# chhylp123/BitMapperBS

Hardware: AMD Instinct MI355X
Metric: M 150bp PE reads aligned/s (higher is better)
Workload: dtype u64

## Files before the change

### bitmapperbs_amd/csrc/bmbs_api.hip

```cpp
#include "bmbs_host.h"
#include "bmbs_kernels.hip"



int ensure(Lane* c, DevBuf& b, size_t bytes, bool zero)
{
    if (bytes == 0) bytes = 16;
    if (b.cap >= bytes) return BMBS_OK;
    size_t want = bytes + bytes / 8 + 256;
    if (c->kn.arena && want <= ((size_t)256 << 20)) {
        if (b.cap) want = std::min<size_t>(std::max(want, b.cap + b.cap / 2), (size_t)256 << 20);
        void* p = c->arena.alloc(want);
        if (!p) { c->err = "out of device memory (lane arena)"; return BMBS_ENOMEM; }
        if (b.p && !b.arena) (void)hipFree(b.p);
        b.p = p; b.cap = want; b.arena = true;
    } else {
        if (b.p && !b.arena) (void)hipFree(b.p);
        b.p = nullptr; b.cap = 0; b.arena = false;
        hipError_t e = hipMalloc(&b.p, want);
        if (e != hipSuccess) { c->err = std::string("hipMalloc: ") + hipGetErrorString(e); b.p = nullptr; return BMBS_ENOMEM; }
        b.cap = want;
    }
    if (zero && hipMemsetAsync(b.p, 0, want, c->stream) != hipSuccess) { c->err = "hipMemsetAsync failed"; return BMBS_ESTATE; }
    return BMBS_OK;
// ... 916 lines not shown
    prof_begin(c, "k_reduce");
    HIPCHK(c, hipMemsetAsync(st.job_flag, 0, n * 4, c->stream));
    HIPCHK(c, hipMemsetAsync(st.red_status, 0, n, c->stream));
    hipLaunchKernelGGL(k_reduce, dim3(nblk(n, 256)), dim3(256), 0, c->stream, (long)n, c->prm.ambiguous_out, st, c->vote_off.as<u64>(),
                       c->votes_dense.as<bmbs_vote>(), c->ferr.as<u32>(), c->fend.as<int>(), tot_at(c, TOT_VOTE_READS), c->vote_list.as<u32>());
    prof_end(c);
    return BMBS_OK;
}

int map_se_dev(Lane* c, const Pending& P)
{
    ReadGeom gm = {};
    int max_ops = 0;
    int rc = call_open(c, P, (u64)P.n, &gm, &max_ops);
    if (rc || P.n == 0) return rc;
    const u64 n = (u64)P.n;
    const char* d_seq = reinterpret_cast<const char*>(P.a[0]);
    const char* d_qual = reinterpret_cast<const char*>(P.a[1]);
    if (P.packed_hw) {
        ENS(c, c->pk_ascii, n * (u64)P.stride + 64);
        { int rz_ = ensure(c, c->prow, n * (u64)pack_words(gm.L) * 8 + 64, true); if (rz_) return rz_; } ENS(c, c->prow_dirty, n + 64);
        HIPCHK(c, hipMemsetAsync(c->prow_dirty.p, 0, n + 64, c->stream));
        prof_begin(c, "k_rows_from_packed");
        rows_from_packed(c, reinterpret_cast<const u64*>(P.a[0]), P.packed_hw, gm, 0, n, false, c->pk_ascii.as<char>(), P.stride);
        prof_end(c);
        d_seq = c->pk_ascii.as<char>();
    }
    const ReadState st = read_state(c);
    u64 tot = 0;
    rc = run_seed_stages(c, d_seq, gm, P.stride, n, &tot, 0, P.exact, P.packed_hw > 0);
    if (rc) return rc;
    c->last_total_cand = tot;
    rc = se_filter_reduce(c, gm, st, d_seq, P.stride, n, tot, P.exact);
    if (rc) return rc;
    rc = align_jobs(c, P, gm, st, d_seq, d_qual, nullptr, n, 0xffffffffu, max_ops);
    if (rc) return rc;
    prof_begin(c, "k_finalize");
    hipLaunchKernelGGL(k_finalize, dim3(nblk(n, 256)), dim3(256), 0, c->stream, c->ix, c->sp, c->pen_lut.as<int>(),
                       c->mapq_lut.as<u8>(), c->mapq_off.as<u32>(), c->mapq_unit, d_seq, d_qual, gm, P.stride, (long)n, st, c->a_start.as<int>(),
                       c->a_end.as<int>(), c->a_nm.as<u32>(), c->a_score.as<int>(), c->a_nops.as<int>(), max_ops, P.cigar_base,
                       c->prm.ambiguous_out, c->sd_sp0.as<u64>(), c->sd_hits0.as<u32>(),
                       reinterpret_cast<bmbs_result_dev*>(P.d_results), c->call_stats.as<unsigned long long>());
    prof_end(c);
    return call_end(c, P.slot);
}

struct PeCall {
    Lane* c; ReadGeom gm; PeIns pi; ReadState st; PeState ps; PeCand *A, *B; char* seq_all; u64 n, n2; int stride; bool exact; u64 tot;
    bool prepacked;
    int rows(const Pending& P);
    int seed();
    int votes();
    int verify_round(int round, u64 cap, const char* name_f, const char* name_c);
    int verify_fast();
    int verify_sensitive();
};

int PeCall::rows(const Pending& P)
{
    prepacked = false;
    if (P.packed_hw) {
        { int rz_ = ensure(c, c->prow, n2 * (u64)pack_words(gm.L) * 8 + 64, true); if (rz_) return rz_; } ENS(c, c->prow_dirty, n2 + 64);
        HIPCHK(c, hipMemsetAsync(c->prow_dirty.p, 0, n2 + 64, c->stream));
        prof_begin(c, "k_rows_from_packed");
        rows_from_packed(c, reinterpret_cast<const u64*>(P.a[0]), P.packed_hw, gm, 0, n, false, seq_all, stride);
        rows_from_packed(c, reinterpret_cast<const u64*>(P.a[2]), P.packed_hw, gm, n, n, true, seq_all, stride);
        prof_end(c);
        prepacked = true;
    } else if (!P.prepared) {
        u64* prow = nullptr; u32* pdirty = nullptr;
        const int pwords = pack_words(gm.L), W = pack_base_words(gm.L);
        if (use_packed_rows(c)) {
            { int rz_ = ensure(c, c->prow, n2 * (u64)pwords * 8 + 64, true); if (rz_) return rz_; } ENS(c, c->prow_dirty, n2 + 64);
            HIPCHK(c, hipMemsetAsync(c->prow_dirty.p, 0, n2 + 64, c->stream));
            prow = c->prow.as<u64>(); pdirty = c->prow_dirty.as<u32>(); prepacked = true;
        }
        const int sparse = prow != nullptr;
        const char* seq1 = reinterpret_cast<const char*>(P.a[0]);
        const char* seq2 = reinterpret_cast<const char*>(P.a[2]);
        prof_begin(c, "k_pe_prepare");
        const int ppr = stride / 16;
        if (sparse && ppr <= 256) {
            const int rpb = 256 / ppr;
            hipLaunchKernelGGL(k_pe_prepare_p, dim3(std::min<u64>(nblk(n, rpb), 2048)), dim3(256), (size_t)rpb * (ppr + 1) * 16, c->stream,
                               seq1, seq2, gm, stride, (long)n, seq_all, prow, pwords, W, pdirty);
        } else
        hipLaunchKernelGGL(k_pe_prepare, dim3(nblk(n * (stride / 16), 256)), dim3(256), 0, c->stream, seq1, seq2, gm, stride, (long)n, seq_all,
                           prow, pwords, W, pdirty, sparse);
        prof_end(c);
    }
    return BMBS_OK;
}

int PeCall::seed()
{
    ps.occ = c->pe_occ.as<int>(); ps.len = c->pe_len.as<u32>(); ps.cur = c->pe_cur.as<u8>(); ps.vround = c->pe_vround.as<u8>();
    ps.dead = c->pe_dead.as<u8>(); ps.both = c->pe_both.as<u8>(); ps.npair = c->pe_npair.as<int>(); ps.sbd = c->pe_sbd.as<u32>();
    if (c->prm.sensitive) {
        ENS(c, c->pe_first, n); ENS(c, c->pe_full, n2); ENS(c, c->pe_roff, n2 * 8); ENS(c, c->pe_rflag, n * 4); ENS(c, c->pe_rscan, (n + 1) * 8);
        ENS(c, c->pe_rlist, n * 4); ENS(c, c->pe_rcnt, n * 4); ENS(c, c->pe_ritem_off, (n + 1) * 8);
    }
    ps.first = c->pe_first.as<u8>(); ps.full = c->pe_full.as<u8>(); ps.R = c->pe_R.as<PeCand>(); ps.roff = c->pe_roff.as<u64>();
    c->last_reseeded = 0; c->last_reseed_cand = 0;
    int rc = launch_seeding(c, seq_all, gm, stride, n2, 1, prepacked);
    if (rc) return rc;
    prof_begin(c, "scan_cand");
// ... 24 lines not shown
        hipLaunchKernelGGL(k_vote_pe_dense, dim3(nblk(n2, VOTE_DENSE_BLOCK)), dim3(VOTE_DENSE_BLOCK), 0, c->stream, c->ix, (long)n2, gm, st, ps, A, c->long_flag.as<u32>(), mid_flag);
    else
        hipLaunchKernelGGL(k_vote_pe_fused, dim3(nblk(n2, 64)), dim3(64), 0, c->stream, c->ix, (long)n2, gm, st, ps, A, c->long_flag.as<u32>(), mid_flag);
    prof_end(c);
    if (use_mid) {
        prof_begin(c, "k_vote_pe_mid");
        int rc = scan_u32(c, mid_flag, n2, c->long_off.as<u64>(), TOT_MID, c->pe_mid_list.as<u32>());
        if (rc) return rc;
        hipLaunchKernelGGL(k_vote_pe_mid, dim3(nblk(n2, 64)), dim3(64), 0, c->stream, c->ix, gm, st, ps, tot_at(c, TOT_MID), c->pe_mid_list.as<u32>(), A, cnt);
        prof_end(c);
    }
    prof_begin(c, "k_vote_pe_long");
    const int prefilter = (!c->prm.sensitive && c->kn.prefilter) ? 1 : 0;
    int rc = scan_u32(c, c->long_flag.as<u32>(), n2, c->long_off.as<u64>(), TOT_LONG, c->long_list.as<u32>());
    if (rc) return rc;
    ENS(c, c->big_list, n2 * 4 + 64);
    unsigned long long* big_count = c->totals.as<unsigned long long>() + TOT_BIG;
    HIPCHK(c, hipMemsetAsync(big_count, 0, 8, c->stream));
    hipLaunchKernelGGL((k_vote_pe_long<VM_CAP, VM_BLOCK, VOTE_REG>), dim3(32768), dim3(VM_BLOCK), 0, c->stream, c->ix, gm, st, ps,
                       tot_at(c, TOT_LONG), c->long_list.as<u32>(), A, c->big_list.as<u32>(), big_count, c->cand.as<u64>(), cnt, (long)n, pi, prefilter, c->long_flag.as<u32>());
    prof_end(c);
    prof_begin(c, "k_vote_pe_big");
    hipLaunchKernelGGL((k_vote_pe_long<1024, 128, VM_CAP>), dim3(8192), dim3(128), 0, c->stream, c->ix, gm, st, ps,
                       tot_at(c, TOT_BIG), c->big_list.as<u32>(), A, (u32*)nullptr, (unsigned long long*)nullptr, c->cand.as<u64>(), cnt, (long)n, pi, prefilter, c->long_flag.as<u32>());
    hipLaunchKernelGGL((k_vote_pe_long<2048, 256, 1024>), dim3(4096), dim3(256), 0, c->stream, c->ix, gm, st, ps,
                       tot_at(c, TOT_BIG), c->big_list.as<u32>(), A, (u32*)nullptr, (unsigned long long*)nullptr, c->cand.as<u64>(), cnt, (long)n, pi, prefilter, c->long_flag.as<u32>());
    hipLaunchKernelGGL((k_vote_pe_long<VL_CAP, VL_BLOCK, 2048>), dim3(2048), dim3(VL_BLOCK), 0, c->stream, c->ix, gm, st, ps,
                       tot_at(c, TOT_BIG), c->big_list.as<u32>(), A, (u32*)nullptr, (unsigned long long*)nullptr, c->cand.as<u64>(), cnt, (long)n, pi, prefilter, c->long_flag.as<u32>());
    prof_end(c);
    return BMBS_OK;
}

int PeCall::verify_round(int round, u64 cap, const char* name_f, const char* name_c)
{
    if (cap) {
        prof_begin(c, name_f);
        u32* wcnt = c->sd_flag_c.as<u32>();
        u64* woff = c->sd_off_c.as<u64>();
        hipLaunchKernelGGL(k_pe_count, dim3(nblk(n2, 256)), dim3(256), 0, c->stream, (long)n, (long)n2, round, ps, wcnt);
        int rc = scan_u32(c, wcnt, n2, woff, TOT_PE_WORK);
        if (rc) return rc;
        hipLaunchKernelGGL(k_pe_worklist, dim3(nblk(n2, 256)), dim3(256), 0, c->stream, (long)n2, wcnt, woff, c->dense_read.as<u32>(),
                           c->ferr.as<u32>());
        hipLaunchKernelGGL(k_filter_pe, dim3(nblk(cap, 256)), dim3(256), 0, c->stream, c->ix, seq_all, packed_rows(c, gm), gm, stride, st, ps, A, B,
                           tot_at(c, TOT_PE_WORK), c->dense_read.as<u32>(), c->ferr.as<u32>(), c->counters.as<unsigned long long>());
        prof_end(c);
    }
    prof_begin(c, name_c);
    hipLaunchKernelGGL(k_pe_compact, dim3(nblk(n2, 64)), dim3(64), 0, c->stream, (long)n, (long)n2, gm, round, st, ps, A, B);
    prof_end(c);
    return BMBS_OK;
}

int PeCall::verify_fast()
{
    prof_begin(c, "k_pe_filter_pairs");
    u32* pef_flag = (c->kn.pef_long == 2 || (c->kn.pef_long == 1 && c->lr_long > 0.005)) ? c->long_flag.as<u32>() : nullptr;
    if (pef_flag) HIPCHK(c, hipMemsetAsync(pef_flag, 0, n * 4, c->stream));
    hipLaunchKernelGGL(k_pe_filter_pairs, dim3(nblk(n, 64)), dim3(64), 0, c->stream, (long)n, gm, pi, st, ps, A, B, pef_flag,
                       c->counters.as<unsigned long long>());
    if (pef_flag) {
        int rc = scan_u32(c, pef_flag, n, c->long_off.as<u64>(), TOT_PEF_LONG, c->long_list.as<u32>());
        if (rc) return rc;
        hipLaunchKernelGGL(k_pe_filter_pairs_long, dim3((unsigned)std::min<u64>(n, 65536)), dim3(64), 0, c->stream, (long)n, gm, pi, st, ps, tot_at(c, TOT_PEF_LONG),
                           c->long_list.as<u32>(), A, B);
    }
    prof_end(c);
    int rc = verify_round(1, tot, "k_filter_pe_r1", "k_pe_compact_r1");
    if (rc) return rc;
    prof_begin(c, "k_pe_prune");
    hipLaunchKernelGGL(k_pe_prune, dim3(nblk(n, 64)), dim3(64), 0, c->stream, (long)n, gm, pi, st, ps, A, B);
    prof_end(c);
    return verify_round(2, tot, "k_filter_pe_r2", "k_pe_compact_r2");
}

int PeCall::verify_sensitive()
{
    unsigned long long* cnt = c->counters.as<unsigned long long>();
    prof_begin(c, "k_pes_order");
    hipLaunchKernelGGL(k_pes_order, dim3(nblk(n, 256)), dim3(256), 0, c->stream, (long)n, st, seed_carry(c), ps);
    prof_end(c);
    int rc = verify_round(1, tot, "k_filter_pe_r1", "k_pe_compact_r1");
    if (rc) return rc;
    prof_begin(c, "k_pes_second");
    hipLaunchKernelGGL(k_pes_second, dim3(nblk(n, 64)), dim3(64), 0, c->stream, (long)n, gm, pi, st, ps, A, B);
    prof_end(c);
    rc = verify_round(2, tot, "k_filter_pe_r2", "k_pe_compact_r2");
    if (rc) return rc;
    prof_begin(c, "k_pes_reseed");
    u32* rflag = c->pe_rflag.as<u32>();
    u32* rlist = c->pe_rlist.as<u32>();
    u32* rcnt = c->pe_rcnt.as<u32>();
    u64* n_reseed = tot_at(c, TOT_RESEED);
    hipLaunchKernelGGL(k_pes_reseed_flag, dim3(nblk(n, 256)), dim3(256), 0, c->stream, (long)n, ps, rflag);
    rc = scan_u32(c, rflag, n, c->pe_rscan.as<u64>(), TOT_RESEED, rlist);
    if (rc) return rc;
    HIPCHK(c, hipMemsetAsync(rcnt, 0, n * 4, c->stream));
    {
        const PackedRows prs = packed_rows(c, gm);
        const bool kg = c->ix.occ3 && prs.base && (c->kn.kgram >= 2 || (c->kn.kgram == 1 && c->lr_chain >= 3.0));
        hipLaunchKernelGGL((kg ? k_pes_reseed<true, true> : prs.base ? k_pes_reseed<true> : k_pes_reseed<false>), dim3(nblk(n, 64)), dim3(64), 0, c->stream, c->ix, seq_all, prs, gm, stride,
                           (long)n, n_reseed, rlist, st, ps, rcnt, cnt);
    }
    rc = scan_u32(c, rcnt, n, c->pe_ritem_off.as<u64>(), TOT_RCAND);
    if (rc) return rc;
    prof_end(c);
    u64 rt[2] = {0, 0};
    if (exact) {
        HIPCHK(c, hipMemcpyAsync(rt, tot_at(c, TOT_RESEED), sizeof rt, hipMemcpyDeviceToHost, c->stream));
        HIPCHK(c, hipStreamSynchronize(c->stream));
    } else {
        rt[0] = n; rt[1] = cap_from(c->lr_rcand, n2, c->kn.cap_scale < 1.0 ? 64 : 65536, c->kn.cap_scale);
        hipLaunchKernelGGL(k_guard_rcand, dim3(nblk(n, 256)), dim3(256), 0, c->stream, tot_at(c, TOT_RCAND), rt[1], c->flags.as<u32>(), (long)n, rcnt,
                           c->pe_ritem_off.as<u64>());
        hipLaunchKernelGGL(k_guard_done, dim3(1), dim3(1), 0, c->stream, tot_at(c, TOT_RCAND), c->flags.as<u32>(), BMBS_FLAG_RCAND);
    }
    c->last_reseeded = rt[0]; c->last_reseed_cand = rt[1];
    if (!rt[0]) return BMBS_OK;
    const u64 rtot = exact ? std::max<u64>(rt[1], cap_from((double)rt[1] / (double)n2, n2, 65536)) : (rt[1] ? rt[1] : 1);
    ENS(c, c->pe_R, rtot * sizeof(PeCand)); ENS(c, c->pe_rcand, rtot * 8);
    ENS(c, c->dense_read, rtot * 4); ENS(c, c->ferr, rtot * 4);
    ps.R = c->pe_R.as<PeCand>();
    prof_begin(c, "k_pes_vote");
    u32* pv_flag = c->long_flag.as<u32>();
    hipLaunchKernelGGL(k_pes_vote, dim3(nblk(rt[0], 64)), dim3(64), 0, c->stream, c->ix, (long)n, gm, pi, n_reseed, rlist,
                       c->pe_ritem_off.as<u64>(), st, ps, c->pe_rcand.as<u64>(), A, B, pv_flag, cnt);
// ... 901 lines not shown
```

### bitmapperbs_amd/csrc/bmbs_host.h

```cpp
#ifndef BMBS_HOST_H
#define BMBS_HOST_H
#include "../../include/bmbs.h"
#include "bmbs_dev.h"
#include <algorithm>
#include <atomic>
#include <cmath>
#include <cstdio>
#include <cstring>
#include <ctime>
#include <sys/syscall.h>
#include <unistd.h>
#include <deque>
#include <memory>
#include <mutex>
#include <string>
#include <thread>
#include <vector>


struct DevBuf {
    void* p = nullptr; size_t cap = 0;
    bool arena = false;
    template <class T> T* as() const { return reinterpret_cast<T*>(p); }
};

struct Arena {
    struct Slab { char* p; size_t cap, used; };
    std::vector<Slab> slabs;
    size_t total = 0;
    void* alloc(size_t bytes)
    {
        bytes = (bytes + 255) & ~(size_t)255;
        for (size_t i = slabs.size(); i-- > 0;)
            if (slabs[i].used + bytes <= slabs[i].cap) { void* r = slabs[i].p + slabs[i].used; slabs[i].used += bytes; return r; }
        size_t cap = std::max<size_t>(bytes, std::min<size_t>((size_t)2 << 30, std::max<size_t>((size_t)512 << 20, total / 2)));
        void* p = nullptr;
        if (hipMalloc(&p, cap) != hipSuccess) {
            cap = bytes;
            if (hipMalloc(&p, cap) != hipSuccess) return nullptr;
        }
        slabs.push_back({(char*)p, cap, bytes});
        total += cap;
        return p;
    }
    void free_all() { for (auto& s : slabs) (void)hipFree(s.p); slabs.clear(); total = 0; }
};

struct Prof { const char* name; hipEvent_t a, b; bool used; };

struct Knobs {
    int sw_form = 0;
    bool rows_ascii = false;
    int seed_waves = 65536;
    bool exact = false;
    int lanes = 3;
    int host_lanes = 4;
    long chunk = 0;
    long split_min = 250000;
    int up_turns = 1;
    int scan_chain = 0;
    int prefilter = 1;
    int pef_long = 1;
    int vote_dense = 1;
    int kgram = 1;
    int seed_stage = 1;
    double cap_scale = 1.0;
    static const bool copy_streams = true, copy_lock = true, arena = true;
    void read()
    {
        auto is = [](const char* e, const char* v) { return e && !strcmp(e, v); };
        const char* e = getenv("BMBS_SW");
        sw_form = is(e, "reg") ? 1 : is(e, "reg2") ? 2 : is(e, "wave") ? 3 : 0;
        rows_ascii = is(getenv("BMBS_LEGACY"), "1");
        if ((e = getenv("BMBS_SEED_WAVES"))) seed_waves = atoi(e);
        exact = is(getenv("BMBS_EXACT"), "1");
        if ((e = getenv("BMBS_LANES"))) lanes = atoi(e);
        if (lanes < 1) lanes = 1;
        if (lanes > 8) lanes = 8;
        if ((e = getenv("BMBS_HOST_LANES"))) host_lanes = atoi(e);
        if (host_lanes < lanes) host_lanes = lanes;
        if (host_lanes > 8) host_lanes = 8;
        if ((e = getenv("BMBS_KGRAM"))) kgram = atoi(e);
        if ((e = getenv("BMBS_CHUNK"))) chunk = atol(e);
        if ((e = getenv("BMBS_SPLIT_MIN"))) split_min = atol(e);
        if (split_min < 1) split_min = 1;
        if ((e = getenv("BMBS_CAP_SCALE"))) cap_scale = atof(e);
        if ((e = getenv("BMBS_PEF_LONG"))) pef_long = atoi(e);
        if ((e = getenv("BMBS_PREFILTER"))) prefilter = atoi(e);
        if ((e = getenv("BMBS_VOTE_DENSE"))) vote_dense = atoi(e);
        if ((e = getenv("BMBS_UP_TURNS"))) up_turns = atoi(e);
        if ((e = getenv("BMBS_SCAN_CHAIN"))) scan_chain = atoi(e);
        if ((e = getenv("BMBS_SEED_STAGE"))) seed_stage = atoi(e) == 0 ? 0 : 1;
    }
};

struct Pending {
    bool pe = false, exact = false;
    int slot = 0;
    uint64_t a[4] = {0, 0, 0, 0};
    const u16* d_len = nullptr;
    int32_t L = 0, stride = 0;
    int64_t n = 0;
    uint64_t d_results = 0, d_cigar_pool = 0;
    int64_t cigar_cap = 0;
    u32 cigar_base = 0;
    bool prepared = false;
    int packed_hw = 0;
    bool staged = false;
};

struct Occ3Shared {
    std::mutex mu;
    bool tried = false;
    int skipped = 0;
    int dev = 0;
    DevIndex base;
    u64 rows = 0;
    void* occ3 = nullptr; void* c3 = nullptr; u64 nb3 = 0;
    ~Occ3Shared() { if (occ3 || c3) { (void)hipSetDevice(dev); if (occ3) (void)hipFree(occ3); if (c3) (void)hipFree(c3); } }
};

struct RecIn { DevBuf in, len, off; };

struct Lane {
    int dev = 0;
    hipStream_t stream = nullptr;
    hipStream_t up_stream = nullptr, down_stream = nullptr;
    hipEvent_t ev_up = nullptr, ev_k = nullptr;
    bmbs_params prm;
    ScoreParams sp;
    Knobs kn;
    Arena arena;
    std::string err;
    bool attached = false;
    DevIndex ix;
    u64 rows = 0;
    DevBuf occ, hash, sa, gen2, gen2p, chrom_start, t20;
    std::shared_ptr<Occ3Shared> o3;
    DevBuf pen_lut, mapq_lut;
    bool luts_ready = false;
    int mapq_unit = 0;
    DevBuf mapq_off, klut;
// ... 143 lines not shown
```

### bitmapperbs_amd/csrc/k_pe_fast.hip

```cpp
struct PeCand { u64 site; u32 err; int32_t end; };

struct PeIns { int min_ins, max_ins; };
DEVI void pe_bounds(const ReadGeom& gm, const PeIns& pi, long p, long n, long long& maxd, long long& mind, int& large_k)
{
    const int L1 = gm.rl(p), L2 = gm.rl(p + n);
    const int k1 = gm.rk(L1), k2 = gm.rk(L2);
    large_k = k1 > k2 ? k1 : k2;
    maxd = (long long)pi.max_ins + 2LL * large_k;
    mind = (long long)pi.min_ins - 2LL * large_k - (L1 > L2 ? L1 : L2);
}

struct PeState {
    int*  occ;
    u32*  len;
    u8*   cur;
    u8*   vround;
    u8*   dead;
    u8*   both;
    int*  npair;
    u32*  sbd;
    u8*   first;
    u8*   full;
    PeCand* R;
    u64*  roff;
// ... 416 lines not shown
                if (mate_here && turn == 0) __threadfence();
                __syncthreads();
                continue;
            }
            vl_locate_range(ix, st.seeds + (size_t)r * BMBS_MAX_SEEDS, st.n_seeds[r], 0, (int)nc, keys, sh_pref, true);
            int cnt = (int)nc;
            if (prefilter && v == 3) {
                const bool earlier = !listed(m) || (long)st.n_cand[m] <= LO;
                const bool mate_final = (turn == 1 || earlier) && ps.len[m] <= PREF_STAGE;
                long long maxd, mind; int large_k;
                pe_bounds(gm, pi, r < n_pairs ? r : r - n_pairs, n_pairs, maxd, mind, large_k);
                if (mate_final && mind <= 0 && maxd >= 0) {
                    const int occm = ps.occ[m];
                    const long nm = occm == 0 ? 0 : (long)ps.len[m];
                    const PeCand* ml = A + st.cand_off[m];
                    if (nm == 0) cnt = 0;
                    else if (!(ml[nm - 1].site >> 63)) {
                        const int kept = pe_prefilter<EMAX>(keys, cnt, k, ml, nm, (u64)maxd, sh_mate, sh_w);
                        if (kept >= 0) cnt = kept;
                    }
                    if (cnt < (int)nc && counters && threadIdx.x == 0) atomicAdd(&SHARD(counters)[CNT_PREFILTER_DROP], (unsigned long long)(nc - cnt));
                }
            }
            if (cnt == 0) {
                if (threadIdx.x == 0) { ps.occ[r] = -1; ps.len[r] = 0; }
                __syncthreads();
                continue;
            }
            vl_sort_keys<EMAX>(keys, cnt);
            if (v == 4) {
                for (long i = threadIdx.x; i < cnt; i += BLOCK) { PeCand e; e.site = keys[i]; e.err = 0; e.end = L - 1; o[i] = e; }
                if (threadIdx.x == 0) { ps.occ[r] = (int)cnt; ps.len[r] = (u32)cnt; }
            } else {
                const int nv = vl_run_ends(keys, cnt, endpos, sh_w);
                for (int e2 = threadIdx.x; e2 < nv; e2 += BLOCK) {
                    const u64 site = keys[endpos[e2]];
                    PeCand e; e.site = site < (u64)k ? 0 : site - (u64)k; e.err = 0; e.end = 0;
                    o[e2] = e;
                }
                if (threadIdx.x == 0) { ps.occ[r] = -1; ps.len[r] = (u32)nv; }
            }
            if (mate_here && turn == 0) __threadfence();
            __syncthreads();
        }
    }
}

DEVI PeCand* pe_list(const PeState& ps, const ReadState& st, PeCand* A, PeCand* B, long r)
{
    const int cur = ps.cur[r];
    return cur == 2 ? ps.R + ps.roff[r] : (cur ? B : A) + st.cand_off[r];
}

DEVI void pe_filter_decide(const PeState& ps, long p, long r1, long r2, int occ1, int occ2, long la, long lb)
{
    ps.cur[r1] = 1; ps.cur[r2] = 1;
    ps.len[r1] = (u32)la; ps.len[r2] = (u32)lb;
    if (la == 0 || lb == 0) { ps.dead[p] = 1; return; }
    if (occ1 == -1 && occ2 == -1) {
        ps.both[p] = 1;
        if (la <= lb) { ps.vround[r1] = 1; ps.vround[r2] = 2; } else { ps.vround[r2] = 1; ps.vround[r1] = 2; }
    } else if (occ1 != -1) {
        if (la < occ1) ps.occ[r1] = (int)la;
        ps.vround[r2] = 1;
    } else {
        if (lb < occ2) ps.occ[r2] = (int)lb;
        ps.vround[r1] = 1;
    }
}
DEVI void pe_filter_serial(const PeCand* a, long na, const PeCand* b, long nb, long long maxd, long long mind, PeCand* ra, PeCand* rb, long& la_out, long& lb_out)
{
    long la = 0, lb = 0, first = 0;
    for (long i = 0; i < na; i++) {
        for (long j = first; j < nb; j++) {
            bool hit = false;
            if (a[i].site > b[j].site) {
                const long long d = (long long)(a[i].site - b[j].site);
                if (d > maxd) first = j + 1;
                else if (d >= mind) hit = true;
            } else {
                const long long d = (long long)(b[j].site - a[i].site);
                if (d > maxd) break;
                if (d >= mind) hit = true;
            }
            if (hit) {
                if (la == 0 || a[i].site > ra[la - 1].site) ra[la++] = a[i];
                if (lb == 0 || b[j].site > rb[lb - 1].site) rb[lb++] = b[j];
            }
        }
    }
    la_out = la; lb_out = lb;
}
#define PEF_LONG 24
__global__ void __launch_bounds__(64)
k_pe_filter_pairs(long n, ReadGeom gm, PeIns pi, ReadState st, PeState ps, PeCand* __restrict__ A, PeCand* __restrict__ B, u32* __restrict__ long_flag,
                  unsigned long long* __restrict__ counters)
{
    const long p = (long)blockIdx.x * blockDim.x + threadIdx.x;
    const long r1 = p, r2 = p + n;
    int occ1 = 1, occ2 = 1;
    if (p < n) {
        occ1 = ps.occ[r1]; occ2 = ps.occ[r2];
        ps.dead[p] = 0; ps.both[p] = 0; ps.npair[p] = 0; ps.sbd[p] = 0;
    }
    const bool runs = p < n && !(occ1 > 0 && occ2 > 0) && occ1 != 0 && occ2 != 0;
    const long na = runs ? (long)ps.len[r1] : 0, nb = runs ? (long)ps.len[r2] : 0;
    wave_count_add(counters, CNT_PEF_ENTRIES, (u32)(na + nb));
    if (p >= n) return;
    long long maxd, mind; int large_k;
    pe_bounds(gm, pi, p, n, maxd, mind, large_k);
    if (occ1 > 0 && occ2 > 0) return;
    if (occ1 == 0 || occ2 == 0) { ps.dead[p] = 1; return; }
    if (long_flag && na + nb > PEF_LONG) { long_flag[p] = 1; return; }
    long la, lb;
    pe_filter_serial(A + st.cand_off[r1], na, A + st.cand_off[r2], nb, maxd, mind, B + st.cand_off[r1], B + st.cand_off[r2], la, lb);
    pe_filter_decide(ps, p, r1, r2, occ1, occ2, la, lb);
}

DEVI long pe_lower_bound(const PeCand* v, long n, u64 key)
{
    long lo = 0, hi = n;
    while (lo < hi) { const long mid = (lo + hi) >> 1; if (v[mid].site < key) lo = mid + 1; else hi = mid; }
    return lo;
}
DEVI long pe_filter_side(const PeCand* x, long nx, const PeCand* y, long ny, u64 maxd, PeCand* out)
{
    const int lane = threadIdx.x & 63;
    long w = 0;
    for (long base = 0; base < nx; base += 64) {
        const long i = base + lane;
        bool keep = false;
        PeCand e; e.site = 0; e.err = 0; e.end = 0;
        if (i < nx) {
            e = x[i];
            const long j = pe_lower_bound(y, ny, e.site > maxd ? e.site - maxd : 0);
            keep = j < ny && (y[j].site <= e.site || y[j].site - e.site <= maxd);
            if (keep && i > 0 && x[i - 1].site == e.site) keep = false;
        }
        const unsigned long long m = __ballot(keep);
        if (keep) out[w + __popcll(m & ((1ull << lane) - 1))] = e;
        w += __popcll(m);
    }
    return w;
}
__global__ void __launch_bounds__(64)
k_pe_filter_pairs_long(long n, ReadGeom gm, PeIns pi, ReadState st, PeState ps, const u64* __restrict__ count_ptr, const u32* __restrict__ list,
                       PeCand* __restrict__ A, PeCand* __restrict__ B)
{
    const long total = (long)*count_ptr;
    for (long item = blockIdx.x; item < total; item += gridDim.x) {
        const long p = list[item];
        long long maxd, mind; int large_k;
        pe_bounds(gm, pi, p, n, maxd, mind, large_k);
        const long r1 = p, r2 = p + n;
        const int occ1 = ps.occ[r1], occ2 = ps.occ[r2];
        const PeCand* a = A + st.cand_off[r1];
        const PeCand* b = A + st.cand_off[r2];
        PeCand* ra = B + st.cand_off[r1];
        PeCand* rb = B + st.cand_off[r2];
        const long na = ps.len[r1], nb = ps.len[r2];
        long la = 0, lb = 0;
        const bool wrapped = (na && (a[na - 1].site >> 63)) || (nb && (b[nb - 1].site >> 63));
        if (mind <= 0 && maxd >= 0 && !wrapped) {
            la = pe_filter_side(a, na, b, nb, (u64)maxd, ra);
            lb = pe_filter_side(b, nb, a, na, (u64)maxd, rb);
        } else {
            if ((threadIdx.x & 63) == 0) pe_filter_serial(a, na, b, nb, maxd, mind, ra, rb, la, lb);
            la = __shfl((int)la, 0, 64); lb = __shfl((int)lb, 0, 64);
        }
        if ((threadIdx.x & 63) == 0) pe_filter_decide(ps, p, r1, r2, occ1, occ2, la, lb);
    }
}

__global__ void __launch_bounds__(256)
k_pe_count(long n, long n2, int round, PeState ps, u32* __restrict__ cnt)
{
    const long r = (long)blockIdx.x * blockDim.x + threadIdx.x;
    if (r >= n2) return;
    const long p = r < n ? r : r - n;
    cnt[r] = (ps.vround[r] == round && !ps.dead[p]) ? ps.len[r] : 0u;
}
__global__ void __launch_bounds__(256)
k_pe_worklist(long n2, const u32* __restrict__ cnt, const u64* __restrict__ off, u32* __restrict__ work_r, u32* __restrict__ work_i)
{
    const long r = (long)blockIdx.x * blockDim.x + threadIdx.x;
    if (r >= n2) return;
    const u32 m = cnt[r];
    const u64 o = off[r];
    for (u32 i = 0; i < m; i++) { work_r[o + i] = (u32)r; work_i[o + i] = i; }
}
__global__ void __launch_bounds__(256)
k_filter_pe(DevIndex ix, const char* __restrict__ seq, PackedRows pr, ReadGeom gm, int stride, ReadState st, PeState ps,
            PeCand* __restrict__ A, PeCand* __restrict__ B, const u64* __restrict__ n_work, const u32* __restrict__ work_r,
            const u32* __restrict__ work_i, unsigned long long* __restrict__ counters)
{
    const u64 g = (u64)blockIdx.x * blockDim.x + threadIdx.x;
    if (g >= *n_work) return;
    const long r = (long)work_r[g];
    PeCand* e = pe_list(ps, st, A, B, r) + work_i[g];
    u32 er; int es;
    const int L = gm.rl(r), k = gm.rk(L);
    bpm_read(ix, seq, stride, pr, r, L, k, e->site, er, es);
    e->err = er; e->end = es;
    if (counters) atomicAdd(&SHARD(counters)[3], 1ull);
}

__global__ void __launch_bounds__(64)
k_pe_compact(long n, long n2, ReadGeom gm, int round, ReadState st, PeState ps, PeCand* __restrict__ A, PeCand* __restrict__ B)
{
    const long r = (long)blockIdx.x * blockDim.x + threadIdx.x;
    const int lane = threadIdx.x & 63;
    bool act = r < n2 && ps.vround[r] == round;
    if (act) { const long p = r < n ? r : r - n; if (ps.dead[p]) act = false; }
    const long m = act ? (long)ps.len[r] : 0;
    const bool coop = m > 64;
    if (act && !coop) {
        const int k = gm.rk(gm.rl(r));
        PeCand* l = pe_list(ps, st, A, B, r);
        u64 pre = ~0ull;
        int occ = 0;
        for (long i = 0; i < m; i++) {
            const PeCand c = l[i];
            const u64 t = c.site + (u64)(long long)c.end;
            if (c.err <= (u32)k && pre != t) { l[occ] = c; occ++; }
            pre = t;
        }
        ps.occ[r] = occ;
    }
    unsigned long long todo = __ballot(coop);
    while (todo) {
        const int src = __ffsll((long long)todo) - 1;
        todo &= todo - 1;
        const long rr = (long)__shfl((long long)r, src, 64);
        const long mm = (long)ps.len[rr];
        const int k = gm.rk(gm.rl(rr));
        PeCand* l = pe_list(ps, st, A, B, rr);
        u64 carry = ~0ull;
        int occ = 0;
        for (long base = 0; base < mm; base += 64) {
            const long i = base + lane;
            PeCand c; c.site = 0; c.err = 0; c.end = 0;
            u64 t = 0;
            if (i < mm) { c = l[i]; t = c.site + (u64)(long long)c.end; }
            u64 pre = (u64)__shfl_up((long long)t, 1, 64);
            if (lane == 0) pre = carry;
            const bool keep = i < mm && c.err <= (u32)k && pre != t;
            const unsigned long long kb = __ballot(keep);
            if (keep) l[occ + __popcll(kb & ((1ull << lane) - 1))] = c;
            occ += __popcll(kb);
            carry = (u64)__shfl((long long)t, 63, 64);
        }
        if (lane == src) ps.occ[rr] = occ;
    }
}

__global__ void __launch_bounds__(64)
k_pe_prune(long n, ReadGeom gm, PeIns pi, ReadState st, PeState ps, PeCand* __restrict__ A, PeCand* __restrict__ B)
{
    const long p = (long)blockIdx.x * blockDim.x + threadIdx.x;
    const int lane = threadIdx.x & 63;
    bool act = p < n && !ps.dead[p] && ps.both[p];
    long long maxd = 0, mind = 0; int large_k;
    long rs = 0, ro = 0;
    int occ_s = 0;
    if (act) {
        pe_bounds(gm, pi, p, n, maxd, mind, large_k);
        rs = ps.vround[p] == 1 ? p : p + n;
        ro = ps.vround[p] == 1 ? p + n : p;
        occ_s = ps.occ[rs];
        if (occ_s == 0) { ps.dead[p] = 1; act = false; }
    }
    const long nb = act ? (long)ps.len[ro] : 0;
    auto serial = [&](const PeCand* a, long na, PeCand* b, long nbb, long long mxd, long long mnd) -> long {
        long len2 = 0, first = 0;
        for (long i = 0; i < na; i++) {
            for (long j = first; j < nbb; j++) {
                if (a[i].site > b[j].site) {
                    const long long d = (long long)(a[i].site - b[j].site);
                    if (d > mxd) first = j + 1;
                    else if (d >= mnd) { b[len2] = b[j]; len2++; first = j + 1; }
                } else {
                    const long long d = (long long)(b[j].site - a[i].site);
                    if (d > mxd) break;
                    if (d >= mnd) { b[len2] = b[j]; len2++; first = j + 1; }
                }
            }
        }
        return len2;
    };
    const bool coop = act && nb + occ_s > 64 && mind <= 0 && maxd >= 0;
    if (act && !coop) ps.len[ro] = (u32)serial(pe_list(ps, st, A, B, rs), occ_s, pe_list(ps, st, A, B, ro), nb, maxd, mind);
    unsigned long long todo = __ballot(coop);
    while (todo) {
        const int src = __ffsll((long long)todo) - 1;
        todo &= todo - 1;
        const long pp = (long)__shfl((long long)p, src, 64);
        long long mxd, mnd; int lk;
        pe_bounds(gm, pi, pp, n, mxd, mnd, lk);
        const long rs2 = ps.vround[pp] == 1 ? pp : pp + n, ro2 = ps.vround[pp] == 1 ? pp + n : pp;
        const long na = ps.occ[rs2], nbb = (long)ps.len[ro2];
        const PeCand* a = pe_list(ps, st, A, B, rs2);
        PeCand* b = pe_list(ps, st, A, B, ro2);
        if ((a[na - 1].site >> 63) || (nbb && (b[nbb - 1].site >> 63))) {
            if (lane == src) ps.len[ro2] = (u32)serial(a, na, b, nbb, mxd, mnd);
            continue;
        }
        long len2 = 0;
        for (long base = 0; base < nbb; base += 64) {
            const long j = base + lane;
            PeCand e; e.site = 0; e.err = 0; e.end = 0;
            bool keep = false;
            if (j < nbb) {
                e = b[j];
                const long i = pe_lower_bound(a, na, e.site > (u64)mxd ? e.site - (u64)mxd : 0);
                keep = i < na && (a[i].site <= e.site || a[i].site - e.site <= (u64)mxd);
            }
            const unsigned long long kb = __ballot(keep);
            if (keep) b[len2 + __popcll(kb & ((1ull << lane) - 1))] = e;
            len2 += __popcll(kb);
        }
        if (lane == src) ps.len[ro2] = (u32)len2;
    }
}
```

### bitmapperbs_amd/csrc/k_scan.hip

```cpp
#define SCAN_BLOCK 256
#define SCAN_ITEMS 8
DEVI u64 block_scan_incl(u64 v, u64* sh_waves, u64& total)
{
    const int lane = threadIdx.x & 63, w = threadIdx.x >> 6, nw = (blockDim.x + 63) >> 6;
    for (int d = 1; d < 64; d <<= 1) { const u64 t = __shfl_up(v, d); if (lane >= d) v += t; }
    if (lane == 63) sh_waves[w] = v;
    __syncthreads();
    u64 add = 0, tot = 0;
    for (int i = 0; i < nw; i++) { const u64 x = sh_waves[i]; if (i < w) add += x; tot += x; }
    __syncthreads();
    total = tot;
    return v + add;
}
DEVI void scan_load8(const u32* in, u64 base, u64 n, u32 x[SCAN_ITEMS])
{
    if (base + SCAN_ITEMS <= n) {
        const uint4 a = *reinterpret_cast<const uint4*>(in + base), b = *reinterpret_cast<const uint4*>(in + base + 4);
        x[0] = a.x; x[1] = a.y; x[2] = a.z; x[3] = a.w; x[4] = b.x; x[5] = b.y; x[6] = b.z; x[7] = b.w;
    } else {
#pragma unroll
        for (int j = 0; j < SCAN_ITEMS; j++) x[j] = base + j < n ? in[base + j] : 0u;
    }
}
__global__ void __launch_bounds__(SCAN_BLOCK) k_scan_partial(const u32* in, u64 n, u64* block_sums, int nz, const u64* __restrict__ n_dev)
{
    __shared__ u64 sh[SCAN_BLOCK / 64];
    if (n_dev) { const u64 nd = *n_dev; if (nd < n) n = nd; }
    const u64 base = (u64)blockIdx.x * SCAN_BLOCK * SCAN_ITEMS + (u64)threadIdx.x * SCAN_ITEMS;
    u32 x[SCAN_ITEMS];
    scan_load8(in, base, n, x);
    if (nz) {
#pragma unroll
        for (int j = 0; j < SCAN_ITEMS; j++) x[j] = x[j] != 0;
    }
    u64 s = 0;
#pragma unroll
    for (int j = 0; j < SCAN_ITEMS; j++) s += x[j];
    u64 total;
    (void)block_scan_incl(s, sh, total);
    if (threadIdx.x == 0) block_sums[blockIdx.x] = total;
}
__global__ void __launch_bounds__(SCAN_BLOCK) k_scan_final(const u32* in, u64 n, const u64* __restrict__ block_sums, u64* out, u32* list, int nz, const u64* __restrict__ n_dev, u64* total)
{
    __shared__ u64 sh[SCAN_BLOCK / 64];
    if (n_dev) { const u64 nd = *n_dev; if (nd < n) n = nd; }
    const u64 base = (u64)blockIdx.x * SCAN_BLOCK * SCAN_ITEMS + (u64)threadIdx.x * SCAN_ITEMS;
    u32 x[SCAN_ITEMS];
    scan_load8(in, base, n, x);
    if (nz) {
#pragma unroll
        for (int j = 0; j < SCAN_ITEMS; j++) x[j] = x[j] != 0;
    }
    u64 s = 0;
#pragma unroll
    for (int j = 0; j < SCAN_ITEMS; j++) s += x[j];
    u64 before = 0;
    for (u32 i = threadIdx.x; i < blockIdx.x; i += SCAN_BLOCK) before += block_sums[i];
    u64 prefix;
    (void)block_scan_incl(before, sh, prefix);
    u64 tot;
    const u64 incl = block_scan_incl(s, sh, tot);
    if (blockIdx.x == gridDim.x - 1 && threadIdx.x == 0) *total = prefix + tot;
    u64 run = incl - s + prefix;
    if (list) {
#pragma unroll
        for (int j = 0; j < SCAN_ITEMS; j++) if (base + j < n && x[j]) { list[run] = (u32)(base + j); run += x[j]; }
        return;
    }
    if (base + SCAN_ITEMS <= n) {
        u64 o[SCAN_ITEMS];
#pragma unroll
        for (int j = 0; j < SCAN_ITEMS; j++) { o[j] = run; run += x[j]; }
        ulonglong2* dst = reinterpret_cast<ulonglong2*>(out + base);
#pragma unroll
        for (int j = 0; j < SCAN_ITEMS; j += 2) dst[j >> 1] = make_ulonglong2(o[j], o[j + 1]);
    } else {
#pragma unroll
        for (int j = 0; j < SCAN_ITEMS; j++) if (base + j < n) { out[base + j] = run; run += x[j]; }
    }
    if (base <= n && n < base + SCAN_ITEMS) out[n] = run;
    if (n % ((u64)SCAN_BLOCK * SCAN_ITEMS) == 0 && n && base + SCAN_ITEMS == n) out[n] = run;
}
#define SCAN_VAL_BITS 38
#define SCAN_VAL_MASK ((1ull << SCAN_VAL_BITS) - 1)
#define SCAN_EPOCH_MAX (1u << 24)
#define SCAN_SUB 4
DEVI u64 scan_word(u32 epoch, u32 state, u64 v) { return ((u64)epoch << (SCAN_VAL_BITS + 2)) | ((u64)state << SCAN_VAL_BITS) | (v & SCAN_VAL_MASK); }
DEVI void block_scan_incl_sub(u64 v[SCAN_SUB], u64 (*sh_waves)[SCAN_BLOCK / 64], u64 tot[SCAN_SUB])
{
    const int lane = threadIdx.x & 63, w = threadIdx.x >> 6;
#pragma unroll
    for (int q = 0; q < SCAN_SUB; q++) {
        for (int d = 1; d < 64; d <<= 1) { const u64 t = __shfl_up(v[q], d); if (lane >= d) v[q] += t; }
        if (lane == 63) sh_waves[q][w] = v[q];
    }
    __syncthreads();
#pragma unroll
    for (int q = 0; q < SCAN_SUB; q++) {
        u64 add = 0, t = 0;
#pragma unroll
        for (int i = 0; i < SCAN_BLOCK / 64; i++) { const u64 x = sh_waves[q][i]; if (i < w) add += x; t += x; }
        v[q] += add; tot[q] = t;
    }
}
__global__ void __launch_bounds__(SCAN_BLOCK) k_scan_chain(const u32* in, u64 n, u64* out, u32* list, int nz, const u64* __restrict__ n_dev, u64* total,
                                                           unsigned int* ticket, u32 ticket_base, u64* status, u32 epoch)
{
    __shared__ u64 sh[SCAN_SUB][SCAN_BLOCK / 64];
    __shared__ u32 sh_tile;
    __shared__ u64 sh_prefix;
    if (n_dev) { const u64 nd = *n_dev; if (nd < n) n = nd; }
    if (threadIdx.x == 0) sh_tile = atomicAdd(ticket, 1u) - ticket_base;
    __syncthreads();
    const u32 tile = sh_tile;
    const u64 base0 = (u64)tile * SCAN_SUB * SCAN_BLOCK * SCAN_ITEMS + (u64)threadIdx.x * SCAN_ITEMS;
    u32 x[SCAN_SUB][SCAN_ITEMS];
    u64 s[SCAN_SUB], incl[SCAN_SUB], tot[SCAN_SUB];
#pragma unroll
    for (int q = 0; q < SCAN_SUB; q++) {
        scan_load8(in, base0 + (u64)q * SCAN_BLOCK * SCAN_ITEMS, n, x[q]);
        if (nz) {
#pragma unroll
            for (int j = 0; j < SCAN_ITEMS; j++) x[q][j] = x[q][j] != 0;
        }
        s[q] = 0;
#pragma unroll
        for (int j = 0; j < SCAN_ITEMS; j++) s[q] += x[q][j];
        incl[q] = s[q];
    }
    block_scan_incl_sub(incl, sh, tot);
    u64 all = 0;
#pragma unroll
    for (int q = 0; q < SCAN_SUB; q++) all += tot[q];
    if (threadIdx.x == 0)
// ... 53 lines not shown
```

Before: 1469.

## Emit per-pair verify counts from filter/prune kernels and build worklists over pairs

The pair filter and prune kernels now write a per-pair count of candidates to verify in the coming round. A two-kernel scan-and-expand over the n pairs then builds the verify worklist directly, instead of a separate count kernel plus a scan over all 2n reads. Compaction likewise runs one thread per pair rather than per read. This removes a count pass and halves the scan and compact domains, at the cost of extra count stores and a serial per-item expansion loop that can be unbalanced when counts are large.

```diff
diff --git a/bitmapperbs_amd/csrc/bmbs_api.hip b/bitmapperbs_amd/csrc/bmbs_api.hip
--- a/bitmapperbs_amd/csrc/bmbs_api.hip
+++ b/bitmapperbs_amd/csrc/bmbs_api.hip
@@ -992,6 +992,7 @@
     int seed();
     int votes();
     int verify_round(int round, u64 cap, const char* name_f, const char* name_c);
+    int verify_round_pairs(int round, u64 cap, const u32* cnt, const char* name_f, const char* name_c);
     int verify_fast();
     int verify_sensitive();
 };
@@ -1122,26 +1123,48 @@
     return BMBS_OK;
 }
 
+int PeCall::verify_round_pairs(int round, u64 cap, const u32* cnt, const char* name_f, const char* name_c)
+{
+    if (cap) {
+        prof_begin(c, name_f);
+        const u64 per = (u64)SCAN_BLOCK * SCAN_ITEMS;
+        const u64 nb = n ? (n + per - 1) / per : 1;
+        { int rc = ensure(c, c->scan_tmp, (nb + 1) * 8, c->kn.scan_chain != 0); if (rc) return rc; }
+        u64* bs = c->scan_tmp.as<u64>();
+        hipLaunchKernelGGL(k_scan_partial, dim3((unsigned)nb), dim3(SCAN_BLOCK), 0, c->stream, cnt, n, bs, 0, (const u64*)nullptr);
+        hipLaunchKernelGGL(k_scan_expand, dim3((unsigned)nb), dim3(SCAN_BLOCK), 0, c->stream, cnt, n, bs, ps.vround, round,
+                           c->dense_read.as<u32>(), c->ferr.as<u32>(), tot_at(c, TOT_PE_WORK));
+        hipLaunchKernelGGL(k_filter_pe, dim3(nblk(cap, 256)), dim3(256), 0, c->stream, c->ix, seq_all, packed_rows(c, gm), gm, stride, st, ps, A, B,
+                           tot_at(c, TOT_PE_WORK), c->dense_read.as<u32>(), c->ferr.as<u32>(), c->counters.as<unsigned long long>());
+        prof_end(c);
+    }
+    prof_begin(c, name_c);
+    hipLaunchKernelGGL(k_pe_compact_pair, dim3(nblk(n, 64)), dim3(64), 0, c->stream, (long)n, gm, round, st, ps, A, B);
+    prof_end(c);
+    return BMBS_OK;
+}
+
 int PeCall::verify_fast()
 {
+    u32* rcnt = c->kn.pe_rounds ? c->sd_flag_c.as<u32>() : nullptr;
     prof_begin(c, "k_pe_filter_pairs");
     u32* pef_flag = (c->kn.pef_long == 2 || (c->kn.pef_long == 1 && c->lr_long > 0.005)) ? c->long_flag.as<u32>() : nullptr;
     if (pef_flag) HIPCHK(c, hipMemsetAsync(pef_flag, 0, n * 4, c->stream));
     hipLaunchKernelGGL(k_pe_filter_pairs, dim3(nblk(n, 64)), dim3(64), 0, c->stream, (long)n, gm, pi, st, ps, A, B, pef_flag,
-                       c->counters.as<unsigned long long>());
+                       c->counters.as<unsigned long long>(), rcnt);
     if (pef_flag) {
         int rc = scan_u32(c, pef_flag, n, c->long_off.as<u64>(), TOT_PEF_LONG, c->long_list.as<u32>());
         if (rc) return rc;
         hipLaunchKernelGGL(k_pe_filter_pairs_long, dim3((unsigned)std::min<u64>(n, 65536)), dim3(64), 0, c->stream, (long)n, gm, pi, st, ps, tot_at(c, TOT_PEF_LONG),
-                           c->long_list.as<u32>(), A, B);
-    }
-    prof_end(c);
-    int rc = verify_round(1, tot, "k_filter_pe_r1", "k_pe_compact_r1");
+                           c->long_list.as<u32>(), A, B, rcnt);
+    }
+    prof_end(c);
+    int rc = rcnt ? verify_round_pairs(1, tot, rcnt, "k_filter_pe_r1", "k_pe_compact_r1") : verify_round(1, tot, "k_filter_pe_r1", "k_pe_compact_r1");
     if (rc) return rc;
     prof_begin(c, "k_pe_prune");
-    hipLaunchKernelGGL(k_pe_prune, dim3(nblk(n, 64)), dim3(64), 0, c->stream, (long)n, gm, pi, st, ps, A, B);
-    prof_end(c);
-    return verify_round(2, tot, "k_filter_pe_r2", "k_pe_compact_r2");
+    hipLaunchKernelGGL(k_pe_prune, dim3(nblk(n, 64)), dim3(64), 0, c->stream, (long)n, gm, pi, st, ps, A, B, rcnt);
+    prof_end(c);
+    return rcnt ? verify_round_pairs(2, tot, rcnt, "k_filter_pe_r2", "k_pe_compact_r2") : verify_round(2, tot, "k_filter_pe_r2", "k_pe_compact_r2");
 }
 
 int PeCall::verify_sensitive()
diff --git a/bitmapperbs_amd/csrc/bmbs_host.h b/bitmapperbs_amd/csrc/bmbs_host.h
--- a/bitmapperbs_amd/csrc/bmbs_host.h
+++ b/bitmapperbs_amd/csrc/bmbs_host.h
@@ -62,6 +62,7 @@
     int prefilter = 1;
     int pef_long = 1;
     int vote_dense = 1;
+    int pe_rounds = 1;
     int kgram = 1;
     int seed_stage = 1;
     double cap_scale = 1.0;
@@ -88,6 +89,7 @@
         if ((e = getenv("BMBS_PEF_LONG"))) pef_long = atoi(e);
         if ((e = getenv("BMBS_PREFILTER"))) prefilter = atoi(e);
         if ((e = getenv("BMBS_VOTE_DENSE"))) vote_dense = atoi(e);
+        if ((e = getenv("BMBS_PE_ROUNDS"))) pe_rounds = atoi(e) == 0 ? 0 : 1;
         if ((e = getenv("BMBS_UP_TURNS"))) up_turns = atoi(e);
         if ((e = getenv("BMBS_SCAN_CHAIN"))) scan_chain = atoi(e);
         if ((e = getenv("BMBS_SEED_STAGE"))) seed_stage = atoi(e) == 0 ? 0 : 1;
diff --git a/bitmapperbs_amd/csrc/k_pe_fast.hip b/bitmapperbs_amd/csrc/k_pe_fast.hip
--- a/bitmapperbs_amd/csrc/k_pe_fast.hip
+++ b/bitmapperbs_amd/csrc/k_pe_fast.hip
@@ -492,21 +492,26 @@
     return cur == 2 ? ps.R + ps.roff[r] : (cur ? B : A) + st.cand_off[r];
 }
 
-DEVI void pe_filter_decide(const PeState& ps, long p, long r1, long r2, int occ1, int occ2, long la, long lb)
+DEVI void pe_filter_decide(const PeState& ps, long p, long r1, long r2, int occ1, int occ2, long la, long lb, u32* __restrict__ cnt1)
 {
     ps.cur[r1] = 1; ps.cur[r2] = 1;
     ps.len[r1] = (u32)la; ps.len[r2] = (u32)lb;
     if (la == 0 || lb == 0) { ps.dead[p] = 1; return; }
+    bool first1;
     if (occ1 == -1 && occ2 == -1) {
         ps.both[p] = 1;
-        if (la <= lb) { ps.vround[r1] = 1; ps.vround[r2] = 2; } else { ps.vround[r2] = 1; ps.vround[r1] = 2; }
+        first1 = la <= lb;
+        if (first1) { ps.vround[r1] = 1; ps.vround[r2] = 2; } else { ps.vround[r2] = 1; ps.vround[r1] = 2; }
     } else if (occ1 != -1) {
         if (la < occ1) ps.occ[r1] = (int)la;
         ps.vround[r2] = 1;
+        first1 = false;
     } else {
         if (lb < occ2) ps.occ[r2] = (int)lb;
         ps.vround[r1] = 1;
-    }
+        first1 = true;
+    }
+    if (cnt1) cnt1[p] = (u32)(first1 ? la : lb);
 }
 DEVI void pe_filter_serial(const PeCand* a, long na, const PeCand* b, long nb, long long maxd, long long mind, PeCand* ra, PeCand* rb, long& la_out, long& lb_out)
 {
@@ -534,7 +539,7 @@
 #define PEF_LONG 24
 __global__ void __launch_bounds__(64)
 k_pe_filter_pairs(long n, ReadGeom gm, PeIns pi, ReadState st, PeState ps, PeCand* __restrict__ A, PeCand* __restrict__ B, u32* __restrict__ long_flag,
-                  unsigned long long* __restrict__ counters)
+                  unsigned long long* __restrict__ counters, u32* __restrict__ cnt1)
 {
     const long p = (long)blockIdx.x * blockDim.x + threadIdx.x;
     const long r1 = p, r2 = p + n;
@@ -542,6 +547,7 @@
     if (p < n) {
         occ1 = ps.occ[r1]; occ2 = ps.occ[r2];
         ps.dead[p] = 0; ps.both[p] = 0; ps.npair[p] = 0; ps.sbd[p] = 0;
+        if (cnt1) cnt1[p] = 0;
     }
     const bool runs = p < n && !(occ1 > 0 && occ2 > 0) && occ1 != 0 && occ2 != 0;
     const long na = runs ? (long)ps.len[r1] : 0, nb = runs ? (long)ps.len[r2] : 0;
@@ -554,7 +560,7 @@
     if (long_flag && na + nb > PEF_LONG) { long_flag[p] = 1; return; }
     long la, lb;
     pe_filter_serial(A + st.cand_off[r1], na, A + st.cand_off[r2], nb, maxd, mind, B + st.cand_off[r1], B + st.cand_off[r2], la, lb);
-    pe_filter_decide(ps, p, r1, r2, occ1, occ2, la, lb);
+    pe_filter_decide(ps, p, r1, r2, occ1, occ2, la, lb, cnt1);
 }
 
 DEVI long pe_lower_bound(const PeCand* v, long n, u64 key)
@@ -585,7 +591,7 @@
 }
 __global__ void __launch_bounds__(64)
 k_pe_filter_pairs_long(long n, ReadGeom gm, PeIns pi, ReadState st, PeState ps, const u64* __restrict__ count_ptr, const u32* __restrict__ list,
-                       PeCand* __restrict__ A, PeCand* __restrict__ B)
+                       PeCand* __restrict__ A, PeCand* __restrict__ B, u32* __restrict__ cnt1)
 {
     const long total = (long)*count_ptr;
     for (long item = blockIdx.x; item < total; item += gridDim.x) {
@@ -608,7 +614,7 @@
             if ((threadIdx.x & 63) == 0) pe_filter_serial(a, na, b, nb, maxd, mind, ra, rb, la, lb);
             la = __shfl((int)la, 0, 64); lb = __shfl((int)lb, 0, 64);
         }
-        if ((threadIdx.x & 63) == 0) pe_filter_decide(ps, p, r1, r2, occ1, occ2, la, lb);
+        if ((threadIdx.x & 63) == 0) pe_filter_decide(ps, p, r1, r2, occ1, occ2, la, lb, cnt1);
     }
 }
 
@@ -645,13 +651,9 @@
     if (counters) atomicAdd(&SHARD(counters)[3], 1ull);
 }
 
-__global__ void __launch_bounds__(64)
-k_pe_compact(long n, long n2, ReadGeom gm, int round, ReadState st, PeState ps, PeCand* __restrict__ A, PeCand* __restrict__ B)
-{
-    const long r = (long)blockIdx.x * blockDim.x + threadIdx.x;
+DEVI void pe_compact_lists(long r, bool act, const ReadGeom& gm, const ReadState& st, const PeState& ps, PeCand* __restrict__ A, PeCand* __restrict__ B)
+{
     const int lane = threadIdx.x & 63;
-    bool act = r < n2 && ps.vround[r] == round;
-    if (act) { const long p = r < n ? r : r - n; if (ps.dead[p]) act = false; }
     const long m = act ? (long)ps.len[r] : 0;
     const bool coop = m > 64;
     if (act && !coop) {
@@ -693,9 +695,29 @@
         if (lane == src) ps.occ[rr] = occ;
     }
 }
-
 __global__ void __launch_bounds__(64)
-k_pe_prune(long n, ReadGeom gm, PeIns pi, ReadState st, PeState ps, PeCand* __restrict__ A, PeCand* __restrict__ B)
+k_pe_compact(long n, long n2, ReadGeom gm, int round, ReadState st, PeState ps, PeCand* __restrict__ A, PeCand* __restrict__ B)
+{
+    const long r = (long)blockIdx.x * blockDim.x + threadIdx.x;
+    bool act = r < n2 && ps.vround[r] == round;
+    if (act) { const long p = r < n ? r : r - n; if (ps.dead[p]) act = false; }
+    pe_compact_lists(r, act, gm, st, ps, A, B);
+}
+__global__ void __launch_bounds__(64)
+k_pe_compact_pair(long n, ReadGeom gm, int round, ReadState st, PeState ps, PeCand* __restrict__ A, PeCand* __restrict__ B)
+{
+    const long p = (long)blockIdx.x * blockDim.x + threadIdx.x;
+    long r = p;
+    bool act = false;
+    if (p < n && !ps.dead[p]) {
+        if (ps.vround[p] == round) act = true;
+        else if (ps.vround[p + n] == round) { r = p + n; act = true; }
+    }
+    pe_compact_lists(r, act, gm, st, ps, A, B);
+}
+
+__global__ void __launch_bounds__(64)
+k_pe_prune(long n, ReadGeom gm, PeIns pi, ReadState st, PeState ps, PeCand* __restrict__ A, PeCand* __restrict__ B, u32* __restrict__ cnt2)
 {
     const long p = (long)blockIdx.x * blockDim.x + threadIdx.x;
     const int lane = threadIdx.x & 63;
@@ -729,7 +751,8 @@
         return len2;
     };
     const bool coop = act && nb + occ_s > 64 && mind <= 0 && maxd >= 0;
-    if (act && !coop) ps.len[ro] = (u32)serial(pe_list(ps, st, A, B, rs), occ_s, pe_list(ps, st, A, B, ro), nb, maxd, mind);
+    u32 left = 0;
+    if (act && !coop) { left = (u32)serial(pe_list(ps, st, A, B, rs), occ_s, pe_list(ps, st, A, B, ro), nb, maxd, mind); ps.len[ro] = left; }
     unsigned long long todo = __ballot(coop);
     while (todo) {
         const int src = __ffsll((long long)todo) - 1;
@@ -742,7 +765,7 @@
         const PeCand* a = pe_list(ps, st, A, B, rs2);
         PeCand* b = pe_list(ps, st, A, B, ro2);
         if ((a[na - 1].site >> 63) || (nbb && (b[nbb - 1].site >> 63))) {
-            if (lane == src) ps.len[ro2] = (u32)serial(a, na, b, nbb, mxd, mnd);
+            if (lane == src) { left = (u32)serial(a, na, b, nbb, mxd, mnd); ps.len[ro2] = left; }
             continue;
         }
         long len2 = 0;
@@ -759,6 +782,7 @@
             if (keep) b[len2 + __popcll(kb & ((1ull << lane) - 1))] = e;
             len2 += __popcll(kb);
         }
-        if (lane == src) ps.len[ro2] = (u32)len2;
-    }
-}
+        if (lane == src) { left = (u32)len2; ps.len[ro2] = left; }
+    }
+    if (cnt2 && p < n) cnt2[p] = left;
+}
diff --git a/bitmapperbs_amd/csrc/k_scan.hip b/bitmapperbs_amd/csrc/k_scan.hip
--- a/bitmapperbs_amd/csrc/k_scan.hip
+++ b/bitmapperbs_amd/csrc/k_scan.hip
@@ -40,12 +40,8 @@
     (void)block_scan_incl(s, sh, total);
     if (threadIdx.x == 0) block_sums[blockIdx.x] = total;
 }
-__global__ void __launch_bounds__(SCAN_BLOCK) k_scan_final(const u32* in, u64 n, const u64* __restrict__ block_sums, u64* out, u32* list, int nz, const u64* __restrict__ n_dev, u64* total)
-{
-    __shared__ u64 sh[SCAN_BLOCK / 64];
-    if (n_dev) { const u64 nd = *n_dev; if (nd < n) n = nd; }
-    const u64 base = (u64)blockIdx.x * SCAN_BLOCK * SCAN_ITEMS + (u64)threadIdx.x * SCAN_ITEMS;
-    u32 x[SCAN_ITEMS];
+DEVI u64 scan_final_run(const u32* in, u64 n, const u64* __restrict__ block_sums, int nz, u64 base, u32 x[SCAN_ITEMS], u64* sh, u64* total)
+{
     scan_load8(in, base, n, x);
     if (nz) {
 #pragma unroll
@@ -61,7 +57,15 @@
     u64 tot;
     const u64 incl = block_scan_incl(s, sh, tot);
     if (blockIdx.x == gridDim.x - 1 && threadIdx.x == 0) *total = prefix + tot;
-    u64 run = incl - s + prefix;
+    return incl - s + prefix;
+}
+__global__ void __launch_bounds__(SCAN_BLOCK) k_scan_final(const u32* in, u64 n, const u64* __restrict__ block_sums, u64* out, u32* list, int nz, const u64* __restrict__ n_dev, u64* total)
+{
+    __shared__ u64 sh[SCAN_BLOCK / 64];
+    if (n_dev) { const u64 nd = *n_dev; if (nd < n) n = nd; }
+    const u64 base = (u64)blockIdx.x * SCAN_BLOCK * SCAN_ITEMS + (u64)threadIdx.x * SCAN_ITEMS;
+    u32 x[SCAN_ITEMS];
+    u64 run = scan_final_run(in, n, block_sums, nz, base, x, sh, total);
     if (list) {
 #pragma unroll
         for (int j = 0; j < SCAN_ITEMS; j++) if (base + j < n && x[j]) { list[run] = (u32)(base + j); run += x[j]; }
@@ -80,6 +84,23 @@
     }
     if (base <= n && n < base + SCAN_ITEMS) out[n] = run;
     if (n % ((u64)SCAN_BLOCK * SCAN_ITEMS) == 0 && n && base + SCAN_ITEMS == n) out[n] = run;
+}
+__global__ void __launch_bounds__(SCAN_BLOCK) k_scan_expand(const u32* in, u64 n, const u64* __restrict__ block_sums, const u8* __restrict__ vround, int round,
+                                                            u32* __restrict__ work_r, u32* __restrict__ work_i, u64* total)
+{
+    __shared__ u64 sh[SCAN_BLOCK / 64];
+    const u64 base = (u64)blockIdx.x * SCAN_BLOCK * SCAN_ITEMS + (u64)threadIdx.x * SCAN_ITEMS;
+    u32 x[SCAN_ITEMS];
+    u64 run = scan_final_run(in, n, block_sums, 0, base, x, sh, total);
+#pragma unroll
+    for (int j = 0; j < SCAN_ITEMS; j++) {
+        const u32 m = x[j];
+        if (!m) continue;
+        const u64 p = base + j;
+        const u32 r = (u32)(vround[p] == round ? p : p + n);
+        for (u32 i = 0; i < m; i++) { work_r[run + i] = r; work_i[run + i] = i; }
+        run += m;
+    }
 }
 #define SCAN_VAL_BITS 38
 #define SCAN_VAL_MASK ((1ull << SCAN_VAL_BITS) - 1)
```

After: 1508, median of 6. 2.7% higher.
